# wei-zeng98/piano-a2s

Measured on AMD Instinct MI355X. Metric: training clips/sec (12 s, 5-bar), higher is better.
Workload: dtype f32

## Files before the change

### include/a2s.h

```cpp
#ifndef A2S_H
#define A2S_H
#include <stddef.h>
#include <stdint.h>
#ifdef __cplusplus
extern "C" {
#endif

#define A2S_OK 0
#define A2S_ERR_ARG (-1)
#define A2S_ERR_HIP (-2)
#define A2S_ERR_WORKSPACE (-3)

const char* a2s_last_error(void);
int a2s_version(void);
long long a2s_launch_count(void);

int a2s_gemm_f32(void* stream, int M, int N, int K, float alpha, const float* A, long sAm, long sAk,
                 const float* B, long sBk, long sBn, float beta, float* C, long ldc, const float* bias, int act,
                 int batch, long bsA, long bsB, long bsC, int splitk, float* workspace, size_t workspace_bytes);
int a2s_gemm_f32_affine(void* stream, int M, int N, int K, float alpha, const float* A, long sAm, long sAk, const float* B, long sBk,
                        long sBn, float beta, float* C, long ldc, const float* bias, int act, int batch, long bsA, long bsB, long bsC,
                        int splitk, float* workspace, size_t workspace_bytes, const float* a_scale, const float* a_shift, int a_period,
                        const float* b_scale, const float* b_shift, int b_period);
int a2s_gemm_f32_bnstats(void* stream, int M, int N, int K, const float* A, long sAm, long sAk, const float* B, long sBk, long sBn, float* C, long ldc,
// ... 124 lines not shown
    int* ids_out; long long* lengths_out; float* score_out;
} a2s_beam_args;
int a2s_note_decoder_fwd_beam(void* stream, const a2s_note_dec_args* args, const a2s_beam_args* beam, int* steps_done);
int a2s_beam_step(void* stream, const a2s_beam_args* beam, const float* logits, long ldl, const float* emb, float* xnext, long ldx, float* h, int h_cols,
                  float* q, int q_cols, int* n_done, int* steps_exec, int B, int V, int E, int t, int max_steps, int eos_id);
int a2s_beam_backtrack(void* stream, const a2s_beam_args* beam, float* probs, long probs_bstride, const int* steps_exec, int B, int V, int max_steps, int eos_id);
int a2s_beam_launches(void);
int a2s_note_decoder_fwd_pair(void* stream_upper, void* stream_lower, const a2s_note_dec_args* upper, const a2s_note_dec_args* lower,
                              const int* pair_order, const int* pair_rank, const int* pair_n_active, int* steps_done_upper, int* steps_done_lower);
size_t a2s_note_step_workspace_floats(int H, int E);
size_t a2s_note_decoder_persist_ws_bytes(int n_clips, int R, int steps);
size_t a2s_note_decoder_bwd_persist_ws_bytes(int n_clips);

int a2s_staff_emb_fwd(void* stream, const float* note_emb, const float* const* gru_w, const long long* ids64,
                      const int* ids32, long id_bstride, const long long* lengths, long len_stride, float* out,
                      long ldo, int col0, float* hsave, int R, int maxlen, int E, int S);


int a2s_log_softmax_bwd_rows(void* stream, const float* g, const float* y, long outer_stride, int inner, float* dx,
                             int R, int V, int n_outer, int time_major);
int a2s_gru_gates_bwd(void* stream, const float* dh_a, long lda, const float* dh_b, long ldb, const float* save,
                      const float* hprev, long ldhp, float* dgi, long ldgi, float* dgh, long ldgh, float* dgh2, long ldgh2,
                      float* dhprev, long lddp, int R, int H);
int a2s_attn_step_bwd(void* stream, const float* keys, const float* enc, const float* q, long ldq, const float* v,
                      const float* attw, const float* ctx, long ldctx, const float* dctx_a, long ldda, const float* dctx_b,
                      long lddb, float* dctx_out, long lddo, float* dq, long lddq, float* ds_out, int B, int T, int H, float* workspace);
int a2s_attn_step_bwd_rows(void* stream, const float* keys, const float* enc, const float* q, long ldq, const float* v, const float* attw,
                           const float* ctx, long ldctx, const float* dctx_a, long ldda, const float* dctx_b, long lddb, float* dctx_out,
                           long lddo, float* dq, long lddq, float* ds_out, int R, int T, int H, float* workspace, int n_clips,
                           const int* clip_order, const int* clip_rank, const int* row_until, int n_active, int step);
int a2s_attn_dk_accum(void* stream, const float* keys, const float* q_all, const float* ds_all, const float* v, float* dK,
                      float* dv_partial, int B, int T, int S, int H, const int* row_until, int groups);
int a2s_attn_dk_blocks(int B, int T);
int a2s_col_sum(void* stream, const float* x, long ld, float* out, long rows, int C, float alpha, float beta, float* workspace, size_t workspace_floats);
int a2s_embed_scatter_add(void* stream, float* table_grad, const long long* ids64, const int* ids32, long id_stride,
                          int const_id, const float* g, long ldg, int col0, int R, int E, const uint8_t* keep_mask, float inv_keep);
int a2s_ew_act_bwd(void* stream, const float* g, const float* y, float* dx, long n, int act);

typedef struct a2s_note_dec_bwd_args {
    const float* attn_w; const float* attn_v; const float* w_ih; const float* w_hh;
    const float* keys; const float* enc;
    const float* h; const float* x; const float* q; const float* gates; const float* attw;
    const float* do_all;
    float* dgi_all; float* dgh_all; float* dq_all; float* ds_all; float* dctx_all; float* dx;
    float* dh;
    float* attn_ws;
    float* gemm_ws; size_t gemm_ws_bytes;
    const int* clip_order;
    const int* clip_rank;
    const int* row_until;
    const int* n_active;
    int n_clips;
    const int* m_active;
    const int* row_list;
    const int* n_rows_active;
    int R, T, H, E, steps;
    float* step_ws; size_t step_ws_floats;
    float* persist_ws; size_t persist_ws_bytes;
    const float* w_ih_full;
} a2s_note_dec_bwd_args;
int a2s_note_decoder_bwd(void* stream, const a2s_note_dec_bwd_args* args);
int a2s_note_decoder_bwd_pair(void* stream_upper, void* stream_lower, const a2s_note_dec_bwd_args* upper, const a2s_note_dec_bwd_args* lower,
                              const int* pair_order, const int* pair_rank, const int* pair_n_active);

int a2s_gru_seq_bwd(void* stream, const float* dout, long do_bstride, long do_tstride, const float* out, long out_bstride,
                    long out_tstride, const float* gates, const float* w_hh, const float* dhn, float* dgi_all, float* dgh_shift,
// ... 57 lines not shown
```

### piano_a2s_amd/csrc/a2s_api.hip

```cpp
#define A2S_SWITCHES_IMPL
#include "a2s_internal.h"

thread_local char a2s_err_msg[512] = {0};
long long a2s_launch_counter = 0;

#define ST ((hipStream_t)stream)

extern "C" {

const char* a2s_last_error(void) { return a2s_err_msg; }
int a2s_version(void) { return 1; }
long long a2s_launch_count(void) { return __atomic_load_n(&a2s_launch_counter, __ATOMIC_RELAXED); }

int a2s_gemm_f32(void* stream, int M, int N, int K, float alpha, const float* A, long sAm, long sAk, const float* B, long sBk,
                 long sBn, float beta, float* C, long ldc, const float* bias, int act, int batch, long bsA, long bsB, long bsC,
                 int splitk, float* workspace, size_t workspace_bytes) {
    return a2s_gemm_impl(ST, M, N, K, alpha, A, sAm, sAk, B, sBk, sBn, beta, C, ldc, bias, act, batch, bsA, bsB, bsC, splitk,
                         workspace, workspace_bytes);
}
int a2s_gemm_f32_affine(void* stream, int M, int N, int K, float alpha, const float* A, long sAm, long sAk, const float* B, long sBk,
                        long sBn, float beta, float* C, long ldc, const float* bias, int act, int batch, long bsA, long bsB, long bsC,
                        int splitk, float* workspace, size_t workspace_bytes, const float* a_scale, const float* a_shift, int a_period,
                        const float* b_scale, const float* b_shift, int b_period) {
    return a2s_gemm_affine_impl(ST, M, N, K, alpha, A, sAm, sAk, B, sBk, sBn, beta, C, ldc, bias, act, batch, bsA, bsB, bsC, splitk,
// ... 21 lines not shown
    return a2s_linear_dgrad_bnstats_impl(ST, M, N, K, dz, lda, Wt, 1, K, da, ldc, y, mean, invstd, scale, shift, period, partial, dz_absmax, w_absmax,
                                         workspace, workspace_bytes, da_absmax_out);
}
size_t a2s_linear_dgrad_ws_bytes(int N, int K) { return a2s_linear_dgrad_ws_bytes_impl(N, K); }
int a2s_linear_fwd(void* stream, int M, int N, int K, const float* y, long lda, const float* W, float* z, long ldc, const float* scale, const float* shift,
                   int period, const float* y_absmax, const float* w_absmax, float* workspace, size_t workspace_bytes) {
    return a2s_linear_fwd_impl(ST, M, N, K, y, lda, W, z, ldc, scale, shift, period, y_absmax, w_absmax, workspace, workspace_bytes);
}
int a2s_linear_wgrad(void* stream, int M, int N, int K, const float* dz, long ldz, const float* y, long lda, float* G, long ldg, const float* scale,
                     const float* shift, int period, const float* dz_absmax, const float* y_absmax, float* workspace, size_t workspace_bytes) {
    return a2s_linear_wgrad_impl(ST, M, N, K, dz, ldz, y, lda, G, ldg, scale, shift, period, dz_absmax, y_absmax, workspace, workspace_bytes);
}
size_t a2s_linear_wgrad_ws_bytes(int M, int K) { return a2s_linear_wgrad_ws_bytes_impl(M, K); }
int a2s_linear_wgrad_eligible(int M, int N, int K, int period) { return a2s_linear_wgrad_ok(M, N, K, 256, 4, 4, period, nullptr, nullptr, nullptr) ? 1 : 0; }
int a2s_linear_fwd_eligible(int M, int N, int K, int period) { return a2s_linear_fwd_ok(M, N, K, 4, 4, period, nullptr, nullptr, nullptr) ? 1 : 0; }
int a2s_linear_dgrad_blocks(int M) { return a2s_linear_dgrad_blocks_impl(M); }
int a2s_linear_dgrad_eligible(int M, int N, int K, int period) {
    return a2s_linear_dgrad_ok(M, N, K, 4, 1, K, 4, period, nullptr, nullptr, nullptr, nullptr) ? 1 : 0;
}
int a2s_gemm_f32_bnstats(void* stream, int M, int N, int K, const float* A, long sAm, long sAk, const float* B, long sBk, long sBn, float* C, long ldc,
                         const float* y, const float* mean, const float* invstd, const float* scale, const float* shift, int period, float* partial) {
    return a2s_gemm_affine_impl(ST, M, N, K, 1.f, A, sAm, sAk, B, sBk, sBn, 0.f, C, ldc, nullptr, 0, 1, 0, 0, 0, 1, nullptr, 0,
                                nullptr, nullptr, 0, nullptr, nullptr, 0, y, mean, invstd, scale, shift, partial, period, 0, nullptr, nullptr);
}
int a2s_gemm_bnstats_blocks(int M, int period) { return a2s_cdiv(M, 128) * a2s_gemm_bnstats_slots(period); }
size_t a2s_gemm_workspace_bytes(int M, int N, int batch, int splitk) { return a2s_gemm_workspace_bytes_impl(M, N, batch, splitk); }
int a2s_gemm_pick_splitk(int M, int N, int K, int batch) { return a2s_gemm_pick_splitk_impl(M, N, K, batch); }
void a2s_gemm_debug_tile(int cfg) { a2s_gemm_debug_tile_impl(cfg); }
size_t a2s_note_step_workspace_floats(int H, int E) { return a2s_note_step_workspace_floats_impl(H, E); }
int a2s_debug_set(const char* key, int value) {
    if (!key) return A2S_ERR_ARG;
    const int id = a2s_switch_find(key);
    if (id >= 0) { a2s_switch_store(id, value); return A2S_OK; }
    if (!strcmp(key, "gemm_tile")) { a2s_gemm_debug_tile_impl(value); return A2S_OK; }
    snprintf(a2s_err_msg, sizeof(a2s_err_msg), "a2s_debug_set: unknown key %s", key);
    return A2S_ERR_ARG;
}
int a2s_env_check(void) {
    if (const char* e = a2s_switch_env_error()) A2S_FAIL(A2S_ERR_ARG, "%s: expected a decimal number >= 0", e);
    return A2S_OK;
}

int a2s_persist_abort_latch(void* device_word) { a2s_persist_latch_set(device_word); return A2S_OK; }

int a2s_debug_get(const char* key) {
    if (!key) return -1;
    const int id = a2s_switch_find(key);
    if (id == A2S_SW_attn_pair_fused_rows) return a2s_attn_pair_fused_rows();
    if (id >= 0) return a2s_sw((a2s_switch)id);
    if (!strcmp(key, "attn_pair_launches")) return (int)a2s_attn_pair_launches();
    if (!strcmp(key, "attn_pair_bwd_launches")) return (int)a2s_attn_pair_bwd_launches();
    if (!strcmp(key, "dec_mid_launches")) return a2s_dec_mid_launches();
    if (!strcmp(key, "dec_persist_launches")) return a2s_dec_persist_launches();
    if (!strcmp(key, "edit_distance_launches")) return (int)a2s_edit_distance_launches();
    if (!strcmp(key, "conv_rows16_c20_launches")) return (int)a2s_conv_rows16_c20_launches();
    if (!strcmp(key, "device_cus")) return a2s_device_geometry().cus;
    if (!strcmp(key, "device_xccs")) return a2s_device_geometry().xccs;
    return -1;
}

int a2s_conv3x3(void* stream, const float* x, const float* w, float* y, const float* in_scale, const float* in_shift,
                float* stat_partial, int B, int T, int F, int Cin, int Cout, int flip, float* workspace) {
    return a2s_conv3x3_impl(ST, x, w, y, in_scale, in_shift, stat_partial, B, T, F, Cin, Cout, flip, workspace, nullptr, nullptr, nullptr, nullptr, nullptr, nullptr,
                            nullptr, nullptr);
}
int a2s_conv3x3_ranged(void* stream, const float* x, const float* w, float* y, const float* in_scale, const float* in_shift, const float* in_absmax,
                       float* stat_partial, float* out_absmax, int B, int T, int F, int Cin, int Cout, float* workspace) {
    return a2s_conv3x3_impl(ST, x, w, y, in_scale, in_shift, stat_partial, B, T, F, Cin, Cout, 0, workspace, nullptr, nullptr, nullptr, nullptr, nullptr, nullptr,
                            in_absmax, out_absmax);
}
int a2s_conv3x3_dgrad_bnstats(void* stream, const float* dy, const float* w, float* g, const float* yl, const float* yl_mean, const float* yl_invstd,
                              const float* yl_scale, const float* yl_shift, float* stat_partial, int B, int T, int F, int Cin, int Cout,
                              float* workspace) {
    if (!yl) { snprintf(a2s_err_msg, sizeof(a2s_err_msg), "conv3x3_dgrad_bnstats: yl is required"); return A2S_ERR_ARG; }
    return a2s_conv3x3_impl(ST, dy, w, g, nullptr, nullptr, stat_partial, B, T, F, Cin, Cout, 1, workspace, yl, yl_mean, yl_invstd, yl_scale, yl_shift, nullptr, nullptr, nullptr);
}
int a2s_conv3x3_dgrad_bnstats_scaled(void* stream, const float* dy, const float* w, float* g, const float* yl, const float* yl_mean, const float* yl_invstd,
                                     const float* yl_scale, const float* yl_shift, float* stat_partial, int B, int T, int F, int Cin, int Cout,
                                     float* workspace, const float* dy_absmax) {
    if (!yl) { snprintf(a2s_err_msg, sizeof(a2s_err_msg), "conv3x3_dgrad_bnstats_scaled: yl is required"); return A2S_ERR_ARG; }
    return a2s_conv3x3_impl(ST, dy, w, g, nullptr, nullptr, stat_partial, B, T, F, Cin, Cout, 1, workspace, yl, yl_mean, yl_invstd, yl_scale, yl_shift, dy_absmax, nullptr, nullptr);
}
int a2s_conv3x3_dgrad_bnstats_ranged(void* stream, const float* dy, const float* w, float* g, const float* yl, const float* yl_mean, const float* yl_invstd,
                                     const float* yl_scale, const float* yl_shift, float* stat_partial, int B, int T, int F, int Cin, int Cout,
// ... 100 lines not shown
int a2s_staff_emb_fwd(void* stream, const float* note_emb, const float* const* gru_w, const long long* ids64, const int* ids32,
                      long id_bstride, const long long* lengths, long len_stride, float* out, long ldo, int col0, float* hsave,
                      int R, int maxlen, int E, int S) {
    if (!gru_w) { snprintf(a2s_err_msg, sizeof(a2s_err_msg), "staff_emb_fwd: null weight table"); return A2S_ERR_ARG; }
    return a2s_staff_emb_fwd_impl(ST, note_emb, gru_w, ids64, ids32, id_bstride, lengths, len_stride, out, ldo, col0, hsave, R,
                                  maxlen, E, S);
}

int a2s_log_softmax_bwd_rows(void* stream, const float* g, const float* y, long outer_stride, int inner, float* dx, int R, int V,
                             int n_outer, int time_major) {
    return a2s_log_softmax_bwd_rows_impl(ST, g, y, outer_stride, inner, dx, R, V, n_outer, time_major);
}
int a2s_gru_gates_bwd(void* stream, const float* dh_a, long lda, const float* dh_b, long ldb, const float* save, const float* hprev,
                      long ldhp, float* dgi, long ldgi, float* dgh, long ldgh, float* dgh2, long ldgh2, float* dhprev, long lddp, int R, int H) {
    return a2s_gru_gates_bwd_impl(ST, dh_a, lda, dh_b, ldb, save, hprev, ldhp, dgi, ldgi, dgh, ldgh, dgh2, ldgh2, dhprev, lddp, R, H);
}
int a2s_attn_step_bwd(void* stream, const float* keys, const float* enc, const float* q, long ldq, const float* v, const float* attw,
                      const float* ctx, long ldctx, const float* dctx_a, long ldda, const float* dctx_b, long lddb, float* dctx_out,
                      long lddo, float* dq, long lddq, float* ds_out, int B, int T, int H, float* workspace) {
    return a2s_attn_step_bwd_impl(ST, keys, enc, q, ldq, v, attw, ctx, ldctx, dctx_a, ldda, dctx_b, lddb, dctx_out, lddo, dq, lddq, ds_out, B, T, H, workspace, nullptr);
}
int a2s_attn_step_bwd_rows(void* stream, const float* keys, const float* enc, const float* q, long ldq, const float* v, const float* attw,
                           const float* ctx, long ldctx, const float* dctx_a, long ldda, const float* dctx_b, long lddb, float* dctx_out,
                           long lddo, float* dq, long lddq, float* ds_out, int R, int T, int H, float* workspace, int n_clips,
                           const int* clip_order, const int* clip_rank, const int* row_until, int n_active, int step) {
    a2s_attn_rows rows = {clip_order, clip_rank, row_until, n_clips, n_active, step};
    return a2s_attn_step_bwd_impl(ST, keys, enc, q, ldq, v, attw, ctx, ldctx, dctx_a, ldda, dctx_b, lddb, dctx_out, lddo, dq, lddq, ds_out, R, T, H, workspace, &rows);
}
int a2s_attn_dk_accum(void* stream, const float* keys, const float* q_all, const float* ds_all, const float* v, float* dK,
                      float* dv_partial, int B, int T, int S, int H, const int* row_until, int groups) {
    return a2s_attn_dk_accum_impl(ST, keys, q_all, ds_all, v, dK, dv_partial, B, T, S, H, row_until, groups);
}
int a2s_attn_dk_blocks(int B, int T) { return B * ((T + 15) / 16); }
int a2s_col_sum(void* stream, const float* x, long ld, float* out, long rows, int C, float alpha, float beta, float* workspace, size_t workspace_floats) {
    return a2s_col_sum_impl(ST, x, ld, out, rows, C, alpha, beta, workspace, workspace_floats);
}
int a2s_embed_scatter_add(void* stream, float* table_grad, const long long* ids64, const int* ids32, long id_stride, int const_id,
                          const float* g, long ldg, int col0, int R, int E, const uint8_t* keep_mask, float inv_keep) {
    return a2s_embed_scatter_add_impl(ST, table_grad, ids64, ids32, id_stride, const_id, g, ldg, col0, R, E, keep_mask, inv_keep);
}
int a2s_ew_act_bwd(void* stream, const float* g, const float* y, float* dx, long n, int act) { return a2s_ew_act_bwd_impl(ST, g, y, dx, n, act); }
int a2s_note_decoder_bwd(void* stream, const a2s_note_dec_bwd_args* args) {
    if (!args) { snprintf(a2s_err_msg, sizeof(a2s_err_msg), "note_decoder_bwd: null args"); return A2S_ERR_ARG; }
    return a2s_note_decoder_bwd_impl(ST, *args);
}
int a2s_note_decoder_bwd_pair(void* stream_upper, void* stream_lower, const a2s_note_dec_bwd_args* upper, const a2s_note_dec_bwd_args* lower,
                              const int* pair_order, const int* pair_rank, const int* pair_n_active) {
    if (!upper || !lower) { snprintf(a2s_err_msg, sizeof(a2s_err_msg), "note_decoder_bwd_pair: null args"); return A2S_ERR_ARG; }
    return a2s_note_decoder_bwd_pair_impl((hipStream_t)stream_upper, (hipStream_t)stream_lower, *upper, *lower, pair_order, pair_rank, pair_n_active);
}
int a2s_gru_seq_bwd(void* stream, const float* dout, long do_bstride, long do_tstride, const float* out, long out_bstride, long out_tstride,
                    const float* gates, const float* w_hh, const float* dhn, float* dgi_all, float* dgh_shift, float* dgh_first,
                    float* dhbuf, float* dgh_tmp, int B, int T, int H, int reverse, float* workspace, size_t workspace_bytes) {
    return a2s_gru_seq_bwd_impl(ST, dout, do_bstride, do_tstride, out, out_bstride, out_tstride, gates, w_hh, dhn, dgi_all, dgh_shift,
                                dgh_first, dhbuf, dgh_tmp, B, T, H, reverse, workspace, workspace_bytes);
}
int a2s_staff_emb_bwd(void* stream, const float* note_emb, const float* const* gru_w, float* const* grads, float* note_emb_grad,
                      const long long* ids64, const int* ids32, long id_bstride, const long long* lengths, long len_stride,
                      const float* dout, long lddo, int col0, const float* hsave, int R, int maxlen, int E, int S) {
    if (!gru_w) { snprintf(a2s_err_msg, sizeof(a2s_err_msg), "staff_emb_bwd: null weight table"); return A2S_ERR_ARG; }
    return a2s_staff_emb_bwd_impl(ST, note_emb, gru_w, grads, note_emb_grad, ids64, ids32, id_bstride, lengths, len_stride, dout, lddo,
                                  col0, hsave, R, maxlen, E, S);
}

int a2s_bn_bwd(void* stream, const float* g, const float* x, const float* mean, const float* invstd, const float* scale, const float* shift,
               const uint8_t* keep_mask, float inv_keep, float* dgamma, float* dbeta, float* dx, float* partial, float* c12, long rows, int C, int F) {
// ... 91 lines not shown
```

### piano_a2s_amd/csrc/a2s_bwd.hip

```cpp
#include "a2s_internal.h"

__global__ __launch_bounds__(256) void log_softmax_bwd_rows(const float* __restrict__ g, const float* __restrict__ y,
                                                            long outer_stride, int inner, float* __restrict__ dx,
                                                            int R, int V, int n_outer, int time_major) {
    const int row = blockIdx.x * 4 + (threadIdx.x >> 6), lane = threadIdx.x & 63;
    if (row >= R) return;
    const int ob = row / inner, in = row % inner;
    const float* gr = g + (long)ob * outer_stride + (long)in * V;
    const float* yr = y + (long)ob * outer_stride + (long)in * V;
    float s = 0.f;
    for (int j = lane; j < V; j += 64) s += gr[j];
    s = wave_sum(s);
    const long orow = time_major ? ((long)in * n_outer + ob) : row;
    for (int j = lane; j < V; j += 64) dx[orow * V + j] = gr[j] - expf(yr[j]) * s;
}

int a2s_log_softmax_bwd_rows_impl(hipStream_t st, const float* g, const float* y, long outer_stride, int inner, float* dx,
                                  int R, int V, int n_outer, int time_major) {
    hipLaunchKernelGGL(log_softmax_bwd_rows, dim3(a2s_cdiv(R, 4)), dim3(256), 0, st, g, y, outer_stride, inner, dx, R, V, n_outer, time_major);
    A2S_CHECK_LAUNCH("log_softmax_bwd_rows");
    return A2S_OK;
}

__global__ void gru_gates_bwd(const float* __restrict__ dh_a, long lda, const float* __restrict__ dh_b, long ldb,
// ... 102 lines not shown
        float dvj = 0.f;
        if (j < H) {
#pragma unroll
            for (int i = 0; i < TT; ++i) { kreg[i] = (t0 + i < T) ? Kmat[((long)b * T + t0 + i) * H + j] : 0.f; acc[i] = 0.f; }
        }
        for (int sg = 0; sg < S * groups; ++sg) {
            const int s = sg / groups, grp = sg % groups;
            if (row_until && s >= row_until[grp * B + b]) continue;
            const long row = (long)sg * B + b;
            __syncthreads();
            if (threadIdx.x < TT) dss[threadIdx.x] = (t0 + threadIdx.x < T) ? ds_all[row * T + t0 + threadIdx.x] : 0.f;
            __syncthreads();
            if (j < H) {
                const float eq = exp2x_clamped(q_all[row * H + j]);
#pragma unroll
                for (int i = 0; i < TT; ++i) {
                    const float e = tanh_ek(kreg[i], eq);
                    acc[i] = fmaf(dss[i], 1.f - e * e, acc[i]);
                    dvj = fmaf(dss[i], e, dvj);
                }
            }
        }
        if (j < H) {
            const float vj = v[j];
#pragma unroll
            for (int i = 0; i < TT; ++i)
                if (t0 + i < T) dK[((long)b * T + t0 + i) * H + j] += vj * acc[i];
            dv_partial[(long)blockIdx.x * H + j] = dvj;
        }
        __syncthreads();
    }
}

int a2s_attn_dk_accum_impl(hipStream_t st, const float* Kmat, const float* q_all, const float* ds_all, const float* v,
                           float* dK, float* dv_partial, int B, int T, int S, int H, const int* row_until, int groups) {
    const int nblk = B * a2s_cdiv(T, 16);
    if (groups < 1) groups = 1;
    A2S_REQUIRE(H >= 1, "attn_dk_accum: hidden_size must be positive (got %d)", H);
    const int nth = H >= 256 ? 256 : (H > 128 ? 256 : (H > 64 ? 128 : 64));
    hipLaunchKernelGGL(attn_dk_accum, dim3(nblk), dim3(nth), 0, st, Kmat, q_all, ds_all, v, dK, dv_partial, B, T, S, row_until, groups, H);
    A2S_CHECK_LAUNCH("attn_dk_accum");
    return A2S_OK;
}

__global__ __launch_bounds__(256) void col_sum(const float* __restrict__ x, long ld, float* __restrict__ out, long rows, int C,
                                               float alpha, float beta) {
    const int c = blockIdx.x * 64 + (threadIdx.x & 63);
    const int part = threadIdx.x >> 6;
    __shared__ float red[4][64];
    float s = 0.f;
    if (c < C) for (long r = part; r < rows; r += 4) s += x[r * ld + c];
    red[part][threadIdx.x & 63] = s;
    __syncthreads();
    if (part == 0 && c < C) {
        const float t = red[0][threadIdx.x] + red[1][threadIdx.x] + red[2][threadIdx.x] + red[3][threadIdx.x];
        out[c] = alpha * t + (beta != 0.f ? beta * out[c] : 0.f);
    }
}

__global__ __launch_bounds__(256) void col_sum_partial(const float* __restrict__ x, long ld, float* __restrict__ partial, long rows, int C, long rpb) {
    const int c = blockIdx.x * 64 + (threadIdx.x & 63);
    const int part = threadIdx.x >> 6;
    const long r0 = (long)blockIdx.y * rpb, r1 = min(rows, r0 + rpb);
    __shared__ float red[4][64];
    float s = 0.f;
    if (c < C) for (long r = r0 + part; r < r1; r += 4) s += x[r * ld + c];
    red[part][threadIdx.x & 63] = s;
    __syncthreads();
    if (part == 0 && c < C)
        partial[(long)blockIdx.y * C + c] = red[0][threadIdx.x] + red[1][threadIdx.x] + red[2][threadIdx.x] + red[3][threadIdx.x];
}
// ... 1125 lines not shown
```

### piano_a2s_amd/csrc/a2s_internal.h

```cpp
#pragma once
#include "a2s_common.h"
#include "../../include/a2s.h"
#include "a2s_switches.h"

static inline int a2s_attn_pair_fused_rows(void) {
    const int cap = a2s_sw(A2S_SW_dec_fused_max_rows), v = a2s_sw(A2S_SW_attn_pair_fused_rows);
    return v < cap ? v : cap;
}
static inline unsigned a2s_persist_dbg(void) {
    return (a2s_sw(A2S_SW_persist_force_agent) ? PERSIST_DBG_FORCE_AGENT : 0u) | (a2s_sw(A2S_SW_persist_inject_abort) ? PERSIST_DBG_INJECT_ABORT : 0u);
}

int a2s_absmax_impl(hipStream_t st, const float* x, long n, float* out);
size_t a2s_gemm_workspace_bytes_impl(int M, int N, int batch, int splitk);
int a2s_gemm_pick_splitk_impl(int M, int N, int K, int batch);
int a2s_gemm_bnstats_slots(int period);
void a2s_gemm_debug_tile_impl(int cfg);
int a2s_gemm_affine_impl(hipStream_t st, int M, int N, int K, float alpha, const float* A, long sAm, long sAk,
    const float* B, long sBk, long sBn, float beta, float* C, long ldc, const float* bias, int act,
    int batch, long bsA, long bsB, long bsC, int splitk, float* ws, size_t ws_bytes,
    const float* a_scale, const float* a_shift, int a_period, const float* b_scale, const float* b_shift, int b_period,
    const float* ep_y, const float* ep_mean, const float* ep_invstd, const float* ep_scale, const float* ep_shift,
    float* ep_partial, int ep_period, int two_term, const float* a_absmax, const float* b_absmax);
int a2s_gemm_impl(hipStream_t st, int M, int N, int K, float alpha, const float* A, long sAm, long sAk,
// ... 89 lines not shown
    long ld_dgh2, float* dhz_out, int R, int H);
int a2s_skinny_gemm_acc_impl(hipStream_t st, const float* A, long lda, const float* Bt, long ldb, float* Cm, long ldc, int R, int N, int K);
int a2s_gru_seq_fwd_impl(hipStream_t st, const float* gi_all, long gi_bstride, long gi_tstride, const float* w_hh,
    const float* b_hh, float* out, long out_bstride, long out_tstride, float* hbuf, float* gh,
    float* save, float* hn, int B, int T, int H, int reverse, float* ws, size_t ws_bytes);
int a2s_attn_step_fwd_impl(hipStream_t st, const float* Kmat, const float* enc, const float* q, long ldq, const float* v,
    float* ctx, long ldctx, float* ctx2, long ldctx2, float* attw, int B, int T, int H,
    const int* n_done, int n_rows_total, float* ws, const a2s_attn_rows* rows = nullptr, a2s_attn_deferred* defer = nullptr);
int a2s_log_softmax_rows_impl(hipStream_t st, const float* x, long ldx, float* y, long ldy, int* argmax_out, int R, int V);
int a2s_embed_rows_impl(hipStream_t st, const float* table, const long long* ids64, const int* ids32, long id_stride,
    int const_id, float* out, long ldo, int col0, int R, int E, const uint8_t* drop, float inv_keep);
int a2s_note_decoder_fwd_impl(hipStream_t st, const a2s_note_dec_args& a, int* steps_done);
int a2s_note_decoder_fwd_grammar_impl(hipStream_t st, const a2s_note_dec_args& a, const a2s_grammar_ref& g, int* steps_done);
int a2s_note_decoder_fwd_pair_impl(hipStream_t su, hipStream_t sl, const a2s_note_dec_args& au, const a2s_note_dec_args& al, const int* pair_order,
    const int* pair_rank, const int* pair_n_active, int* done_u, int* done_l);
int a2s_staff_emb_fwd_impl(hipStream_t st, const float* note_emb, const float* const* w ,
    const long long* ids64, const int* ids32, long id_bstride, const long long* lengths,
    long len_stride, float* out, long ldo, int col0, float* hsave, int R, int maxlen, int E, int S);
size_t a2s_attn_workspace_floats_impl(int B, int T, int H, int groups);
size_t a2s_attn_bulk_lds(size_t shm, int n_active, int backward);
long a2s_attn_pair_launches(void);

int a2s_log_softmax_bwd_rows_impl(hipStream_t st, const float* g, const float* y, long outer_stride, int inner, float* dx,
    int R, int V, int n_outer, int time_major);
int a2s_gru_gates_bwd_impl(hipStream_t st, const float* dh_a, long lda, const float* dh_b, long ldb, const float* save,
    const float* hprev, long ldhp, float* dgi, long ldgi, float* dgh, long ldgh, float* dgh2, long ldgh2,
    float* dhprev, long lddp, int R, int H);
int a2s_attn_step_bwd_impl(hipStream_t st, const float* Kmat, const float* enc, const float* q, long ldq, const float* v,
    const float* attw, const float* ctx, long ldctx, const float* dctx_a, long ldda, const float* dctx_b,
    long lddb, float* dctx_out, long lddo, float* dq, long lddq, float* ds_out, int B, int T, int H, float* ws,
    const a2s_attn_rows* rows = nullptr);
int a2s_attn_dk_accum_impl(hipStream_t st, const float* Kmat, const float* q_all, const float* ds_all, const float* v,
    float* dK, float* dv_partial, int B, int T, int S, int H, const int* row_until, int groups);
int a2s_col_sum_impl(hipStream_t st, const float* x, long ld, float* out, long rows, int C, float alpha, float beta, float* ws, size_t ws_floats);
int a2s_embed_scatter_add_impl(hipStream_t st, float* table_grad, const long long* ids64, const int* ids32, long id_stride,
    int const_id, const float* g, long ldg, int col0, int R, int E, const uint8_t* drop, float inv_keep);
int a2s_ew_act_bwd_impl(hipStream_t st, const float* g, const float* y, float* dx, long n, int act);
int a2s_note_decoder_bwd_impl(hipStream_t st, const a2s_note_dec_bwd_args& a);
int a2s_note_decoder_bwd_pair_impl(hipStream_t su, hipStream_t sl, const a2s_note_dec_bwd_args& au, const a2s_note_dec_bwd_args& al, const int* pair_order,
    const int* pair_rank, const int* pair_n_active);
int a2s_gru_seq_bwd_impl(hipStream_t st, const float* dout, long do_bstride, long do_tstride, const float* out, long out_bstride,
    long out_tstride, const float* gates, const float* w_hh, const float* dhn, float* dgi_all, float* dgh_shift,
    float* dgh_first, float* dhbuf, float* dgh_tmp, int B, int T, int H, int reverse, float* ws, size_t ws_bytes);
int a2s_staff_emb_bwd_impl(hipStream_t st, const float* note_emb, const float* const* w, float* const* grads_dev, float* note_emb_grad,
    const long long* ids64, const int* ids32, long id_bstride, const long long* lengths, long len_stride,
    const float* dout, long lddo, int col0, const float* hsave, int R, int maxlen, int E, int S);
long a2s_attn_pair_bwd_launches(void);

size_t a2s_note_step_fused_head_floats(void);
size_t a2s_note_step_workspace_floats_impl(int H, int E);
int a2s_dec_mid_launches(void);
bool a2s_dec_step_fusable(int R, int H, int E, int V, const void* const* ptrs, int nptrs, const float* ws, size_t ws_floats, bool greedy = false);
int a2s_note_step_fused_fwd(hipStream_t st, const a2s_note_dec_args& a, int si, int so, int sv, int sv_next, int t, const int* t_base, int tf, bool last,
    int nrows, const int* rowmap, const a2s_attn_deferred* defer = nullptr);
int a2s_note_step_fused_bwd_prepare(hipStream_t st, const a2s_note_dec_bwd_args& a);
int a2s_note_step_fused_bwd(hipStream_t st, const a2s_note_dec_bwd_args& a, int s, const float* dh_in, float* dh_out, const a2s_attn_rows* rows,
    int nrows, const int* rowmap);
bool a2s_note_step_mid_ok(int H, int E, const void* const* ptrs, int nptrs);
int a2s_note_step_mid_gru(hipStream_t st, const a2s_note_dec_args& a, int si, int so, int sv, int sv_next, int nrows, const int* rowmap);
bool a2s_note_step_mid_bwd_ok(const a2s_note_dec_bwd_args& a);
int a2s_note_step_mid_bwd(hipStream_t st, const a2s_note_dec_bwd_args& a, int s, float* dh_out, int nrows, const int* rowmap);
int a2s_note_step_mid_bwd_query(hipStream_t st, const a2s_note_dec_bwd_args& a, int s, float* dh_out, int nrows, const int* rowmap);

bool a2s_grammar_ref_ok(const a2s_grammar_ref& g, int R, int V);
int a2s_grammar_argmax_rows_impl(hipStream_t st, const float* x, long ldx, float* y, long ldy, const signed char* next, int n_states, int* row_state,
    int* choice_out, int R, int V);
// ... 63 lines not shown
```

### piano_a2s_amd/csrc/a2s_switches.h

```cpp
#pragma once
#include <stdio.h>
#include <stdlib.h>
#include <string.h>

#define A2S_SWITCHES(X)                                                                                                                              \
     \
    X(conv_rows, 7, COUNT, "A2S_CONV_ROWS")                                                                                                          \
                                                                         \
    X(wgrad_rows, 1, COUNT, "A2S_WGRAD_ROWS")                                                                                                        \
             \
    X(conv_c1_fast, 1, RAW, 0)                                                                                                                       \
           \
    X(conv_bf16x3, 3, RAW, 0)                                                                                                                        \
                              \
    X(conv_f16x2, 3, COUNT, 0)                                                                                                                       \
                                  \
    X(wgrad_bf16x3, 1, RAW, 0)                                                                                                                       \
                                                                \
    X(wgrad_f16x2, 1, COUNT, 0)                                                                                                                      \
                                      \
    X(gemm_bf16x3, 1, RAW, 0)                                                                                                                        \
                                      \
    X(gemm_f16x2, 1, COUNT, 0)                                                                                                                       \
                                                                  \
// ... 10 lines not shown
    X(dec_fused_max_rows, 192, COUNT, 0)                                                                                                             \
                  \
    X(attn_pair_fused_rows, 32, RAW, 0)                                                                                                              \
                                             \
    X(dec_mid, 1, ONOFF, 0)                                                                                                                          \
                                          \
    X(dec_persist, 1, ONOFF, "A2S_DEC_PERSIST")                                                                                                      \
                                               \
    X(attn_pair, 1, ONOFF, 0)                                                                                                                        \
                                          \
    X(attn_deep, 24, COUNT, 0)                                                                                                                       \
                                                              \
    X(attn_defer_combine, 1, ONOFF, 0)                                                                                                               \
      \
    X(attn_fused_combine, 0, COUNT, 0)                                                                                                               \
                                          \
    X(attn_nt, 64, COUNT, 0)                                                                                                                         \
             \
    X(attn_bulk_cap, 0, ONOFF, 0)                                                                                                                    \
                                  \
    X(persist_force_agent, 0, ONOFF, 0)                                                                                                              \
                                                                                 \
    X(persist_inject_abort, 0, ONOFF, 0)

enum a2s_switch {
#define X(key, def, rule, env) A2S_SW_##key,
    A2S_SWITCHES(X)
#undef X
    A2S_SW_COUNT
};
extern int a2s_switch_value[A2S_SW_COUNT];
static inline int a2s_sw(a2s_switch id) { return a2s_switch_value[id]; }

int a2s_switch_find(const char* key);
void a2s_switch_store(int id, int value);
const char* a2s_switch_env_error(void);

#ifdef A2S_SWITCHES_IMPL
enum { A2S_RULE_ONOFF, A2S_RULE_COUNT, A2S_RULE_RAW };
struct a2s_switch_desc { const char* key; int rule; const char* env; };
static const a2s_switch_desc a2s_switch_table[A2S_SW_COUNT] = {
#define X(key, def, rule, env) {#key, A2S_RULE_##rule, env},
    A2S_SWITCHES(X)
#undef X
};
int a2s_switch_value[A2S_SW_COUNT] = {
#define X(key, def, rule, env) def,
    A2S_SWITCHES(X)
#undef X
};
static char a2s_switch_bad_env[96] = {0};

int a2s_switch_find(const char* key) {
    for (int i = 0; key && i < A2S_SW_COUNT; ++i)
        if (!strcmp(key, a2s_switch_table[i].key)) return i;
    return -1;
}
void a2s_switch_store(int id, int value) {
    const int rule = a2s_switch_table[id].rule;
    a2s_switch_value[id] = rule == A2S_RULE_ONOFF ? (value ? 1 : 0) : (rule == A2S_RULE_COUNT && value < 0) ? 0 : value;
}
const char* a2s_switch_env_error(void) { return a2s_switch_bad_env[0] ? a2s_switch_bad_env : nullptr; }

__attribute__((constructor(101))) static void a2s_switch_read_env(void) {
    for (int i = 0; i < A2S_SW_COUNT; ++i) {
        const char* e = a2s_switch_table[i].env ? getenv(a2s_switch_table[i].env) : nullptr;
// ... 13 lines not shown
```

### piano_a2s_amd/engine_bwd.py

```python
import ctypes as C
import os
import threading

import torch

from . import hip
from .spec import SOS, VOCAB_SIZE

NULL = C.c_void_p(0)


def _os_env(name, default):
    return os.environ.get(name, default)


def _ptr(t, off=0):
    return C.c_void_p(t.data_ptr() + 4 * off)


_COLSUM_WS = {}


def _colsum(x, ld, out, rows, ncol, x_off=0, out_off=0, beta=1.0):
    ws = None
# ... 16 lines not shown
    if dx is not None:
        hip.gemm(dy, N, 1, W, K, 1, dx, dx.stride(0), M, K, N, beta=dx_beta)
    return dx


_ONES = {}


def _one(dev):
    key = torch.device(dev).index
    if key not in _ONES:
        _ONES[key] = torch.ones(1, dtype=torch.float32, device=dev)
    return _ONES[key]


def _staff_token_bwd(eng, S, G, rec, dtok):
    L = hip.lib()
    names = [f"decoder.staff_emb.{w}_{sfx}" for sfx in ("l0", "l0_reverse") for w in ("weight_ih", "weight_hh", "bias_ih", "bias_hh")]
    warr = (C.c_void_p * 8)(*[S[n].data_ptr() for n in names])
    gptrs = G.get("__staff_emb_ptrs__")
    if gptrs is None:
        gptrs = torch.tensor([G[n].data_ptr() for n in names], dtype=torch.int64, device=dtok.device)
    E, Sz = eng.cfg["note_emb_size"], eng.cfg["staff_emb_size"]
    ids = rec["ids"]
    hip.check(L.a2s_staff_emb_bwd(hip.stream(), hip._p(S["decoder.note_emb.weight"]), warr, hip._p(gptrs), hip._p(G["decoder.note_emb.weight"]),
                                  hip._p(ids) if rec["i64"] else NULL, NULL if rec["i64"] else hip._p(ids), C.c_long(rec["id_bstride"]),
                                  hip._p(rec["lengths"]), C.c_long(rec["len_stride"]), hip._p(dtok), C.c_long(dtok.stride(0)), rec["col0"],
                                  hip._p(rec["hsave"]), dtok.shape[0], rec["maxlen"], E, Sz), "a2s_staff_emb_bwd")
    return gptrs


def _attn_deferred(eng, S, G, prefix, keys, enc, q_all, ds_all, attw_all, dctx_all, dK, dEnc, B, T, H, steps, active=None, groups=1):
    L = hip.lib()
    hip.gemm(attw_all, 1, B * T, dctx_all, B * 2 * H, 1, dEnc, 2 * H, T, 2 * H, steps * groups, beta=1.0, batch=B, bsA=T, bsB=2 * H, bsC=T * 2 * H,
             two_term=(_one(enc.device), hip.absmax(dctx_all)) if dctx_all.is_contiguous() else None)
    nblk = L.a2s_attn_dk_blocks(B, T)
    dvp = torch.empty((nblk, H), dtype=torch.float32, device=enc.device)
    hip.check(L.a2s_attn_dk_accum(hip.stream(), hip._p(keys), hip._p(q_all), hip._p(ds_all), hip._p(S[prefix + ".v.weight"]), hip._p(dK),
                                  hip._p(dvp), B, T, steps, H, hip._p(active["until"] if active else None), groups), "a2s_attn_dk_accum")
    _colsum(dvp, H, G[prefix + ".v.weight"], nblk, H)


def _note_decoder_bwd(eng, S, G, sv, keys, enc, dprobs_bar, probs_bar, dK, dEnc, n_clips, T, deferred=None, enc_amax=None, late=None, defer_launch=False):
    L = hip.lib()
    groups = sv.get("groups", 1)
    B = groups * n_clips
    cfg = eng.cfg
    H, E, V = cfg["hidden_size"], cfg["note_emb_size"], VOCAB_SIZE
    H2, ldx = 2 * H, E + 2 * H
    n, prefix, dev = sv["steps"], sv["prefix"], enc.device
    R = n * B
    dlog = torch.empty((n, B, V), dtype=torch.float32, device=dev)
    hip.check(L.a2s_log_softmax_bwd_rows(hip.stream(), hip._p(dprobs_bar), hip._p(probs_bar), C.c_long(probs_bar.stride(0)), n, hip._p(dlog),
                                         R, V, B, 1), "a2s_log_softmax_bwd_rows")
    o2d, dlog2d = sv["o"].view(R, 2 * H2), dlog.view(R, V)
    do_all = torch.empty((n, B, 2 * H2), dtype=torch.float32, device=dev)
    Wo = S[prefix + ".out.weight"]
    dlog_amax = hip.absmax(dlog) if enc_amax is not None else None
    hip.gemm(dlog2d, V, 1, Wo, 2 * H2, 1, do_all.view(R, 2 * H2), 2 * H2, R, 2 * H2, V,
             two_term=(dlog_amax, hip.absmax(Wo)) if enc_amax is not None else None)
    dgi_all = torch.empty((n, B, 3 * H2), dtype=torch.float32, device=dev)
    dgh_all = torch.empty((n, B, 3 * H2), dtype=torch.float32, device=dev)
    dq_all = torch.empty((n, B, H), dtype=torch.float32, device=dev)
    ds_all = torch.empty((n, B, T), dtype=torch.float32, device=dev)
    dctx_all = torch.empty((n, B, H2), dtype=torch.float32, device=dev)
    m_active = sv["active"].get("m_active") if sv.get("active") else None
    dx = torch.empty((n, B, ldx), dtype=torch.float32, device=dev)
    dh = torch.empty((2, B, H2), dtype=torch.float32, device=dev)
    a = hip.NoteDecBwdArgs()
    for name, t in (("attn_w", S[prefix + ".attn.attn.weight"]), ("attn_v", S[prefix + ".attn.v.weight"]), ("w_ih", S[prefix + ".gru.weight_ih_l0"]),
                    ("w_hh", S[prefix + ".gru.weight_hh_l0"]), ("keys", keys), ("enc", enc), ("h", sv["h"]), ("x", sv["x"]), ("q", sv["q"]),
                    ("gates", sv["gates"]), ("attw", sv["attw"]), ("do_all", do_all), ("dgi_all", dgi_all), ("dgh_all", dgh_all),
# ... 661 lines not shown
```

### piano_a2s_amd/hip.py

```python
import ctypes as C
import os

import torch

from .build import LIB

LIB = os.environ.get("A2S_LIB", LIB)

_lib = None


class A2SError(RuntimeError):
    pass


class NoteDecArgs(C.Structure):
    _fields_ = [(n, C.c_void_p) for n in (
        "attn_w", "attn_b", "attn_v", "w_ih", "w_hh", "b_ih", "b_hh", "out_w", "out_b", "emb", "keys", "enc",
        "h", "x", "q", "gates", "attw", "o", "gh", "gi", "logits")] + [
        ("probs", C.c_void_p), ("probs_bstride", C.c_long),
        ("gt", C.c_void_p), ("gt_bstride", C.c_long),
        ("tf_flags", C.c_void_p),
        ("drop", C.c_void_p), ("inv_keep", C.c_float),
        ("argmax_out", C.c_void_p), ("am_bstride", C.c_long),
# ... 12 lines not shown
        (n, C.c_void_p) for n in ("row_state", "score", "finished", "done_count", "token_hist", "parent_hist", "score_hist", "probs_scratch",
                                  "ids_out", "lengths_out", "score_out")]


class NoteDecBwdArgs(C.Structure):
    _fields_ = [(n, C.c_void_p) for n in (
        "attn_w", "attn_v", "w_ih", "w_hh", "keys", "enc", "h", "x", "q", "gates", "attw", "do_all",
        "dgi_all", "dgh_all", "dq_all", "ds_all", "dctx_all", "dx", "dh", "attn_ws", "gemm_ws")] + [
        ("gemm_ws_bytes", C.c_size_t), ("clip_order", C.c_void_p), ("clip_rank", C.c_void_p), ("row_until", C.c_void_p),
        ("n_active", C.c_void_p), ("n_clips", C.c_int), ("m_active", C.c_void_p), ("row_list", C.c_void_p), ("n_rows_active", C.c_void_p),
        ("R", C.c_int), ("T", C.c_int), ("H", C.c_int), ("E", C.c_int), ("steps", C.c_int),
        ("step_ws", C.c_void_p), ("step_ws_floats", C.c_size_t), ("persist_ws", C.c_void_p), ("persist_ws_bytes", C.c_size_t), ("w_ih_full", C.c_void_p)]


def lib():
    global _lib
    if _lib is None:
        if not os.path.exists(LIB):
            raise A2SError(f"HIP extension not built: {LIB} is missing (run `python __graft_entry__.py build`). "
                           "There is no CPU fallback for the transcription hot path.")
        arith = os.environ.get("A2S_ARITH", "f16x2")
        if arith not in ("f16x2", "bf16x3", "f32"):
            raise A2SError(f"A2S_ARITH={arith!r}: expected f16x2, bf16x3 or f32")
        L = C.CDLL(LIB)
        L.a2s_last_error.restype = C.c_char_p
        L.a2s_launch_count.restype = C.c_longlong
        for fn in ("a2s_note_step_workspace_floats", "a2s_note_decoder_persist_ws_bytes", "a2s_note_decoder_bwd_persist_ws_bytes", "a2s_linear_dgrad_ws_bytes", "a2s_linear_wgrad_ws_bytes", "a2s_gemm_workspace_bytes", "a2s_bn_bwd_partial_floats", "a2s_conv3x3_wgrad_workspace_bytes", "a2s_attn_workspace_floats", "a2s_attn_workspace_floats_fused",
                   "a2s_conv3x3_workspace_floats"):
            getattr(L, fn).restype = C.c_size_t
        if hasattr(L, "a2s_env_check") and L.a2s_env_check() != 0:
            raise A2SError(L.a2s_last_error().decode())
        if hasattr(L, "a2s_edit_distance"):
            L.a2s_edit_distance.argtypes = [C.c_void_p] * 6 + [C.c_int] * 3 + [C.c_void_p]
        if arith != "f16x2":
            for key in (b"conv_f16x2", b"wgrad_f16x2", b"gemm_f16x2"):
                L.a2s_debug_set(key, 0)
        if arith == "f32":
            for key in (b"conv_bf16x3", b"gemm_bf16x3", b"wgrad_bf16x3"):
                L.a2s_debug_set(key, 0)
        _lib = L
    return _lib


LINEAR_KERNELS = os.environ.get("A2S_LINEAR_KERNELS", "1") != "0"

_ABORT_LATCH = {}
PERSIST_ABORTS = 0


def abort_latch(device):
    idx = torch.device(device).index if torch.device(device).index is not None else torch.cuda.current_device()
    t = _ABORT_LATCH.get(idx)
    if t is None:
        t = _ABORT_LATCH[idx] = torch.zeros(1, dtype=torch.int32, device=torch.device("cuda", idx))
        _ABORT_LATCH["registered"] = None
    if _ABORT_LATCH.get("registered") != idx:
        check(lib().a2s_persist_abort_latch(C.c_void_p(t.data_ptr())), "a2s_persist_abort_latch")
        _ABORT_LATCH["registered"] = idx
    return t


_LATCH_READS = {}


def post_persist_abort_read(device):
    idx = torch.device(device).index if torch.device(device).index is not None else torch.cuda.current_device()
# ... 296 lines not shown
```

Before: 617.1.

## Skip inactive decoder steps in deferred attention dK and dEnc accumulation

Adds a live-pair compaction helper that uses a wave ballot to list only the (step, group) rows still active per clip. A new MFMA-based kernel accumulates dEnc from attention weights and context gradients over just those rows, replacing a batched GEMM that covered every step. A prefetching dK accumulation kernel is also added, loading the next chunk of q and ds while the current one is computed. The fast path is enabled by default behind a debug switch, but the dEnc kernel only handles a width of 512 and runs in full f32 instead of the split-precision GEMM path.

```diff
diff --git a/include/a2s.h b/include/a2s.h
--- a/include/a2s.h
+++ b/include/a2s.h
@@ -180,6 +180,8 @@
 int a2s_attn_dk_accum(void* stream, const float* keys, const float* q_all, const float* ds_all, const float* v, float* dK,
                       float* dv_partial, int B, int T, int S, int H, const int* row_until, int groups);
 int a2s_attn_dk_blocks(int B, int T);
+int a2s_attn_denc_accum(void* stream, const float* attw_all, const float* dctx_all, float* dEnc, int B, int T, int S, int H2,
+                        const int* row_until, int groups);
 int a2s_col_sum(void* stream, const float* x, long ld, float* out, long rows, int C, float alpha, float beta, float* workspace, size_t workspace_floats);
 int a2s_embed_scatter_add(void* stream, float* table_grad, const long long* ids64, const int* ids32, long id_stride,
                           int const_id, const float* g, long ldg, int col0, int R, int E, const uint8_t* keep_mask, float inv_keep);
diff --git a/piano_a2s_amd/csrc/a2s_api.hip b/piano_a2s_amd/csrc/a2s_api.hip
--- a/piano_a2s_amd/csrc/a2s_api.hip
+++ b/piano_a2s_amd/csrc/a2s_api.hip
@@ -77,6 +77,7 @@
     if (!key) return A2S_ERR_ARG;
     const int id = a2s_switch_find(key);
     if (id >= 0) { a2s_switch_store(id, value); return A2S_OK; }
+    if (!strcmp(key, "attn_deferred_fast")) { a2s_attn_deferred_fast = value ? 1 : 0; return A2S_OK; }
     if (!strcmp(key, "gemm_tile")) { a2s_gemm_debug_tile_impl(value); return A2S_OK; }
     snprintf(a2s_err_msg, sizeof(a2s_err_msg), "a2s_debug_set: unknown key %s", key);
     return A2S_ERR_ARG;
@@ -95,6 +96,9 @@
     if (id >= 0) return a2s_sw((a2s_switch)id);
     if (!strcmp(key, "attn_pair_launches")) return (int)a2s_attn_pair_launches();
     if (!strcmp(key, "attn_pair_bwd_launches")) return (int)a2s_attn_pair_bwd_launches();
+    if (!strcmp(key, "attn_deferred_fast")) return a2s_attn_deferred_fast;
+    if (!strcmp(key, "attn_dk_ahead_launches")) return (int)a2s_attn_dk_ahead_launches();
+    if (!strcmp(key, "attn_denc_launches")) return (int)a2s_attn_denc_launches();
     if (!strcmp(key, "dec_mid_launches")) return a2s_dec_mid_launches();
     if (!strcmp(key, "dec_persist_launches")) return a2s_dec_persist_launches();
     if (!strcmp(key, "edit_distance_launches")) return (int)a2s_edit_distance_launches();
@@ -261,6 +265,10 @@
     return a2s_attn_dk_accum_impl(ST, keys, q_all, ds_all, v, dK, dv_partial, B, T, S, H, row_until, groups);
 }
 int a2s_attn_dk_blocks(int B, int T) { return B * ((T + 15) / 16); }
+int a2s_attn_denc_accum(void* stream, const float* attw_all, const float* dctx_all, float* dEnc, int B, int T, int S, int H2,
+                        const int* row_until, int groups) {
+    return a2s_attn_denc_accum_impl(ST, attw_all, dctx_all, dEnc, B, T, S, H2, row_until, groups);
+}
 int a2s_col_sum(void* stream, const float* x, long ld, float* out, long rows, int C, float alpha, float beta, float* workspace, size_t workspace_floats) {
     return a2s_col_sum_impl(ST, x, ld, out, rows, C, alpha, beta, workspace, workspace_floats);
 }
diff --git a/piano_a2s_amd/csrc/a2s_bwd.hip b/piano_a2s_amd/csrc/a2s_bwd.hip
--- a/piano_a2s_amd/csrc/a2s_bwd.hip
+++ b/piano_a2s_amd/csrc/a2s_bwd.hip
@@ -158,11 +158,183 @@
     }
 }
 
+constexpr int LIVE_CH = 512;
+__device__ __forceinline__ void live_pairs(int* __restrict__ list, int* __restrict__ cnt, int sg0, int sg1, int b, int B,
+                                           const int* __restrict__ row_until, int groups) {
+    if (threadIdx.x >= 64) return;
+    int n = 0;
+    for (int base = sg0; base < sg1; base += 64) {
+        const int sg = base + (int)threadIdx.x;
+        bool live = sg < sg1;
+        if (live && row_until) live = sg / groups < row_until[(sg % groups) * B + b];
+        const unsigned long long m = __ballot(live);
+        if (live) list[n + __popcll(m & ((1ull << threadIdx.x) - 1ull))] = sg;
+        n += __popcll(m);
+    }
+    if (threadIdx.x == 0) *cnt = n;
+}
+
+#ifndef A2S_ATTN_DK_NS
+#define A2S_ATTN_DK_NS 8
+#endif
+template <int NS>
+__global__ __launch_bounds__(256) void attn_dk_accum_ahead(const float* __restrict__ Kmat, const float* __restrict__ q_all,
+                                                           const float* __restrict__ ds_all, const float* __restrict__ v,
+                                                           float* __restrict__ dK, float* __restrict__ dv_partial, int B, int T, int S,
+                                                           const int* __restrict__ row_until, int groups, int H) {
+    constexpr int TT = 16;
+    static_assert(NS * TT <= 256, "one ds value per thread");
+    const int tiles = (T + TT - 1) / TT;
+    const int b = blockIdx.x / tiles, t0 = (blockIdx.x % tiles) * TT;
+    const int tid = threadIdx.x, j = tid;
+    __shared__ int list[LIVE_CH];
+    __shared__ int cnt_s;
+    __shared__ float dss[2][NS * TT];
+    float kreg[TT], acc[TT];
+    float dvj = 0.f;
+#pragma unroll
+    for (int i = 0; i < TT; ++i) { kreg[i] = (j < H && t0 + i < T) ? Kmat[((long)b * T + t0 + i) * H + j] : 0.f; acc[i] = 0.f; }
+    const int nsg = S * groups, du = tid / TT, di = tid % TT;
+    int buf = 0;
+    for (int c0 = 0; c0 < nsg; c0 += LIVE_CH) {
+        __syncthreads();
+        live_pairs(list, &cnt_s, c0, min(nsg, c0 + LIVE_CH), b, B, row_until, groups);
+        __syncthreads();
+        const int cnt = cnt_s;
+        float qn[NS], dsn = 0.f;
+        auto fetch = [&](int p0) {
+#pragma unroll
+            for (int u = 0; u < NS; ++u) qn[u] = (p0 + u < cnt && j < H) ? q_all[((long)list[p0 + u] * B + b) * H + j] : 0.f;
+            dsn = (tid < NS * TT && p0 + du < cnt && t0 + di < T) ? ds_all[((long)list[p0 + du] * B + b) * T + t0 + di] : 0.f;
+        };
+        fetch(0);
+        for (int p0 = 0; p0 < cnt; p0 += NS) {
+            const int nv = min(NS, cnt - p0);
+            float qc[NS];
+#pragma unroll
+            for (int u = 0; u < NS; ++u) qc[u] = qn[u];
+            if (tid < NS * TT) dss[buf][tid] = dsn;
+            __syncthreads();
+            fetch(p0 + NS);
+            if (j < H) {
+#pragma unroll
+                for (int u = 0; u < NS; ++u) {
+                    if (u < nv) {
+                        const float eq = exp2x_clamped(qc[u]);
+#pragma unroll
+                        for (int i = 0; i < TT; ++i) {
+                            const float e = tanh_ek(kreg[i], eq);
+                            acc[i] = fmaf(dss[buf][u * TT + i], 1.f - e * e, acc[i]);
+                            dvj = fmaf(dss[buf][u * TT + i], e, dvj);
+                        }
+                    }
+                }
+            }
+            buf ^= 1;
+        }
+    }
+    if (j < H) {
+        const float vj = v[j];
+#pragma unroll
+        for (int i = 0; i < TT; ++i)
+            if (t0 + i < T) dK[((long)b * T + t0 + i) * H + j] += vj * acc[i];
+        dv_partial[(long)blockIdx.x * H + j] = dvj;
+    }
+}
+
+int a2s_attn_deferred_fast = 1;
+static long long g_attn_dk_ahead_launches = 0, g_attn_denc_launches = 0;
+long a2s_attn_dk_ahead_launches(void) { return (long)__atomic_load_n(&g_attn_dk_ahead_launches, __ATOMIC_RELAXED); }
+long a2s_attn_denc_launches(void) { return (long)__atomic_load_n(&g_attn_denc_launches, __ATOMIC_RELAXED); }
+
+template <int KB>
+__global__ __launch_bounds__(256, 2) void attn_denc_accum(const float* __restrict__ attw_all, const float* __restrict__ dctx_all,
+                                                       float* __restrict__ dEnc, int B, int T, int S, const int* __restrict__ row_until, int groups) {
+    constexpr int H2 = 512, FT = 64, RT = FT / 16, CT = 8;
+    const int tiles = (T + FT - 1) / FT;
+    const int b = blockIdx.x / tiles, t0 = (blockIdx.x % tiles) * FT;
+    const int wave = threadIdx.x >> 6, lane = threadIdx.x & 63, lk = lane >> 4, lc = lane & 15;
+    const int col0 = wave * (16 * CT);
+    __shared__ int list[LIVE_CH];
+    __shared__ int cnt_s;
+    f32x4 acc[RT][CT];
+#pragma unroll
+    for (int i = 0; i < RT; ++i)
+#pragma unroll
+        for (int c = 0; c < CT; ++c) acc[i][c] = (f32x4){0.f, 0.f, 0.f, 0.f};
+    const int nsg = S * groups;
+    for (int c0 = 0; c0 < nsg; c0 += LIVE_CH) {
+        __syncthreads();
+        live_pairs(list, &cnt_s, c0, min(nsg, c0 + LIVE_CH), b, B, row_until, groups);
+        __syncthreads();
+        const int cnt = cnt_s;
+        float an[KB][RT], bn[KB][CT];
+        auto fetch = [&](int p0) {
+#pragma unroll
+            for (int s = 0; s < KB; ++s) {
+                const int p = p0 + 4 * s + lk;
+                const bool ok = p < cnt;
+                const long row = ok ? (long)list[p] * B + b : 0;
+#pragma unroll
+                for (int i = 0; i < RT; ++i) an[s][i] = (ok && t0 + 16 * i + lc < T) ? attw_all[row * T + t0 + 16 * i + lc] : 0.f;
+#pragma unroll
+                for (int c = 0; c < CT; ++c) bn[s][c] = ok ? dctx_all[row * H2 + col0 + 16 * c + lc] : 0.f;
+            }
+        };
+        fetch(0);
+        for (int p0 = 0; p0 < cnt; p0 += 4 * KB) {
+            float ac[KB][RT], bc[KB][CT];
+#pragma unroll
+            for (int s = 0; s < KB; ++s) {
+#pragma unroll
+                for (int i = 0; i < RT; ++i) ac[s][i] = an[s][i];
+#pragma unroll
+                for (int c = 0; c < CT; ++c) bc[s][c] = bn[s][c];
+            }
+            fetch(p0 + 4 * KB);
+#pragma unroll
+            for (int s = 0; s < KB; ++s)
+#pragma unroll
+                for (int i = 0; i < RT; ++i)
+#pragma unroll
+                    for (int c = 0; c < CT; ++c) acc[i][c] = __builtin_amdgcn_mfma_f32_16x16x4f32(ac[s][i], bc[s][c], acc[i][c], 0, 0, 0);
+        }
+    }
+#pragma unroll
+    for (int i = 0; i < RT; ++i)
+#pragma unroll
+        for (int r = 0; r < 4; ++r) {
+            const int t = t0 + 16 * i + 4 * lk + r;
+            if (t < T) {
+                float* o = dEnc + ((long)b * T + t) * H2 + col0 + lc;
+#pragma unroll
+                for (int c = 0; c < CT; ++c) o[16 * c] += acc[i][c][r];
+            }
+        }
+}
+
+int a2s_attn_denc_accum_impl(hipStream_t st, const float* attw_all, const float* dctx_all, float* dEnc, int B, int T, int S, int H2,
+                             const int* row_until, int groups) {
+    A2S_REQUIRE(H2 == 512, "attn_denc_accum: built for encoder outputs of 512 columns (got %d)", H2);
+    A2S_REQUIRE(B >= 1 && T >= 1 && S >= 0, "attn_denc_accum: B = %d, T = %d, S = %d", B, T, S);
+    if (groups < 1) groups = 1;
+    hipLaunchKernelGGL((attn_denc_accum<2>), dim3(B * a2s_cdiv(T, 64)), dim3(256), 0, st, attw_all, dctx_all, dEnc, B, T, S, row_until, groups);
+    A2S_CHECK_LAUNCH("attn_denc_accum");
+    __atomic_fetch_add(&g_attn_denc_launches, 1LL, __ATOMIC_RELAXED);
+    return A2S_OK;
+}
+
 int a2s_attn_dk_accum_impl(hipStream_t st, const float* Kmat, const float* q_all, const float* ds_all, const float* v,
                            float* dK, float* dv_partial, int B, int T, int S, int H, const int* row_until, int groups) {
     const int nblk = B * a2s_cdiv(T, 16);
     if (groups < 1) groups = 1;
     A2S_REQUIRE(H >= 1, "attn_dk_accum: hidden_size must be positive (got %d)", H);
+    if (a2s_attn_deferred_fast && H <= 256) {
+        hipLaunchKernelGGL((attn_dk_accum_ahead<A2S_ATTN_DK_NS>), dim3(nblk), dim3(256), 0, st, Kmat, q_all, ds_all, v, dK, dv_partial, B, T, S, row_until, groups, H);
+        A2S_CHECK_LAUNCH("attn_dk_accum_ahead");
+        __atomic_fetch_add(&g_attn_dk_ahead_launches, 1LL, __ATOMIC_RELAXED);
+        return A2S_OK;
+    }
     const int nth = H >= 256 ? 256 : (H > 128 ? 256 : (H > 64 ? 128 : 64));
     hipLaunchKernelGGL(attn_dk_accum, dim3(nblk), dim3(nth), 0, st, Kmat, q_all, ds_all, v, dK, dv_partial, B, T, S, row_until, groups, H);
     A2S_CHECK_LAUNCH("attn_dk_accum");
diff --git a/piano_a2s_amd/csrc/a2s_internal.h b/piano_a2s_amd/csrc/a2s_internal.h
--- a/piano_a2s_amd/csrc/a2s_internal.h
+++ b/piano_a2s_amd/csrc/a2s_internal.h
@@ -145,6 +145,10 @@
     const a2s_attn_rows* rows = nullptr);
 int a2s_attn_dk_accum_impl(hipStream_t st, const float* Kmat, const float* q_all, const float* ds_all, const float* v,
     float* dK, float* dv_partial, int B, int T, int S, int H, const int* row_until, int groups);
+int a2s_attn_denc_accum_impl(hipStream_t st, const float* attw_all, const float* dctx_all, float* dEnc, int B, int T, int S, int H2,
+    const int* row_until, int groups);
+long a2s_attn_dk_ahead_launches(void);
+long a2s_attn_denc_launches(void);
 int a2s_col_sum_impl(hipStream_t st, const float* x, long ld, float* out, long rows, int C, float alpha, float beta, float* ws, size_t ws_floats);
 int a2s_embed_scatter_add_impl(hipStream_t st, float* table_grad, const long long* ids64, const int* ids32, long id_stride,
     int const_id, const float* g, long ldg, int col0, int R, int E, const uint8_t* drop, float inv_keep);
diff --git a/piano_a2s_amd/csrc/a2s_switches.h b/piano_a2s_amd/csrc/a2s_switches.h
--- a/piano_a2s_amd/csrc/a2s_switches.h
+++ b/piano_a2s_amd/csrc/a2s_switches.h
@@ -66,6 +66,8 @@
 extern int a2s_switch_value[A2S_SW_COUNT];
 static inline int a2s_sw(a2s_switch id) { return a2s_switch_value[id]; }
 
+extern int a2s_attn_deferred_fast;
+
 int a2s_switch_find(const char* key);
 void a2s_switch_store(int id, int value);
 const char* a2s_switch_env_error(void);
diff --git a/piano_a2s_amd/engine_bwd.py b/piano_a2s_amd/engine_bwd.py
--- a/piano_a2s_amd/engine_bwd.py
+++ b/piano_a2s_amd/engine_bwd.py
@@ -72,12 +72,18 @@
 
 def _attn_deferred(eng, S, G, prefix, keys, enc, q_all, ds_all, attw_all, dctx_all, dK, dEnc, B, T, H, steps, active=None, groups=1):
     L = hip.lib()
-    hip.gemm(attw_all, 1, B * T, dctx_all, B * 2 * H, 1, dEnc, 2 * H, T, 2 * H, steps * groups, beta=1.0, batch=B, bsA=T, bsB=2 * H, bsC=T * 2 * H,
-             two_term=(_one(enc.device), hip.absmax(dctx_all)) if dctx_all.is_contiguous() else None)
+    until = active["until"] if active else None
+    if (2 * H == 512 and L.a2s_debug_get(b"attn_deferred_fast") > 0 and hasattr(L, "a2s_attn_denc_accum")
+            and attw_all.is_contiguous() and dctx_all.is_contiguous() and dEnc.is_contiguous()):
+        hip.check(L.a2s_attn_denc_accum(hip.stream(), hip._p(attw_all), hip._p(dctx_all), hip._p(dEnc), B, T, steps, 2 * H, hip._p(until), groups),
+                  "a2s_attn_denc_accum")
+    else:
+        hip.gemm(attw_all, 1, B * T, dctx_all, B * 2 * H, 1, dEnc, 2 * H, T, 2 * H, steps * groups, beta=1.0, batch=B, bsA=T, bsB=2 * H, bsC=T * 2 * H,
+                 two_term=(_one(enc.device), hip.absmax(dctx_all)) if dctx_all.is_contiguous() else None)
     nblk = L.a2s_attn_dk_blocks(B, T)
     dvp = torch.empty((nblk, H), dtype=torch.float32, device=enc.device)
     hip.check(L.a2s_attn_dk_accum(hip.stream(), hip._p(keys), hip._p(q_all), hip._p(ds_all), hip._p(S[prefix + ".v.weight"]), hip._p(dK),
-                                  hip._p(dvp), B, T, steps, H, hip._p(active["until"] if active else None), groups), "a2s_attn_dk_accum")
+                                  hip._p(dvp), B, T, steps, H, hip._p(until), groups), "a2s_attn_dk_accum")
     _colsum(dvp, H, G[prefix + ".v.weight"], nblk, H)
 
 
diff --git a/piano_a2s_amd/hip.py b/piano_a2s_amd/hip.py
--- a/piano_a2s_amd/hip.py
+++ b/piano_a2s_amd/hip.py
@@ -68,6 +68,8 @@
             raise A2SError(L.a2s_last_error().decode())
         if hasattr(L, "a2s_edit_distance"):
             L.a2s_edit_distance.argtypes = [C.c_void_p] * 6 + [C.c_int] * 3 + [C.c_void_p]
+        if hasattr(L, "a2s_attn_denc_accum"):
+            L.a2s_attn_denc_accum.argtypes = [C.c_void_p] * 4 + [C.c_int] * 4 + [C.c_void_p, C.c_int]
         if arith != "f16x2":
             for key in (b"conv_f16x2", b"wgrad_f16x2", b"gemm_f16x2"):
                 L.a2s_debug_set(key, 0)
```

Measured after the change: 626.5 (median of 6 runs). +1.5%, better.
